# SHI-Labs/Prompt-Free-Diffusion

Hardware: AMD Instinct MI355X
Metric: images/sec @512x512 50-step DDIM, SD-v1.5+SeeCoder (higher is better)
Workload: dtype f16; 1 GPU; [c2] SD-v1.5 UNet + seecoder-v1-0, 512x512, 50-step DDIM (50 real steps), CFG 2.0, fp16, batch=4/GPU, 1 SeeCoder encode(s) + VAE decode per batch; global_batch=4, parallelism=dp1, world_size_reported_by_backend=1, collectives_forced_at_world_1=False

## Files before the change

include/pfd_hip.h:

```cpp
#ifndef PFD_HIP_H
#define PFD_HIP_H

#include <stddef.h>
#include <stdint.h>

#ifdef __cplusplus
extern "C" {
#endif

#define PFD_OK 0
#define PFD_EINVAL (-1)
#define PFD_ESHAPE (-2)
#define PFD_ELAUNCH (-3)

#define PFD_ABI_VERSION 10

typedef void* pfd_stream_t;

#define PFD_ACT_NONE 0
#define PFD_ACT_GELU 1
#define PFD_ACT_RELU 2
#define PFD_ACT_SILU 3
#define PFD_ACT_GEGLU 4

// ... 11 lines not shown
  int32_t M, N, K;
  int32_t rows_per_rv;
  int32_t act;
  int32_t bias_per_row;
  int32_t ksize, stride, pad, ups;
  int32_t B, H, Wd, Cin;
  int32_t Ho, Wo;
  void* ws;
  size_t ws_bytes;
  void* Ct;
  int64_t ldct;
  int32_t n_split;
  int32_t w_tiled;
  const void* gn_table;
  const void* A2;
  int64_t lda2;
  int32_t gn_c1;
  int32_t gn_act;
  const void* ln_stats;
  const void* ln_colsum;
  int32_t ln_parts;
  float ln_eps;
  void* ln_out;
  int32_t k_split;
  int32_t zero_rows;
  void* gn_out;
  const void* gnf_gamma;
  const void* gnf_beta;
  void* gnf_y;
  int64_t gnf_ldy;
  float gnf_eps;
  int32_t gnf_act;
  int32_t gnf_rows;
  int32_t gnf_skip_raw;
  int32_t res_rows;
} PfdGemmDesc;
int pfd_gemm_f16(const PfdGemmDesc* d, pfd_stream_t stream);
int pfd_gemm_f16_ex(const PfdGemmDesc* d, int32_t tile, pfd_stream_t stream);

int32_t pfd_gemm_geglu_group(int32_t N);

typedef struct PfdAttnDesc {
  const void* Q;
  const void* K;
  const void* Vt;
  void* O;
  int64_t ldq, ldk, ldvt, ldo;
  int64_t q_bs, k_bs, vt_bs, o_bs;
  int32_t B, H, Nq, Nk, D;
  float scale;
} PfdAttnDesc;
int pfd_attention_f16(const PfdAttnDesc* d, pfd_stream_t stream);

typedef struct PfdSwinAttnDesc {
  const void* qkv;
  const void* qkv_bias;
  const void* rpb;
  void* out;
  int32_t B, H, W, C, nH, ws, shift;
  float scale;
} PfdSwinAttnDesc;
int pfd_swin_window_attention_f16(const PfdSwinAttnDesc* d, pfd_stream_t stream);

size_t pfd_groupnorm_ws_bytes(int32_t B, int32_t C, int32_t HW);
int32_t pfd_groupnorm_takes_pstats(int32_t B, int32_t C1, int32_t C2, int32_t HW, int32_t G);
int pfd_groupnorm_pstats_f16(const void* x1, int32_t C1, int64_t ldx1, const void* st1, const void* x2, int32_t C2,
                             int64_t ldx2, const void* st2, const void* gamma, const void* beta, void* y, int64_t ldy,
                             int32_t B, int32_t HW, int32_t G, float eps, int32_t act, pfd_stream_t stream);

int pfd_groupnorm_table_f16(const void* x1, int32_t C1, int64_t ldx1, const void* x2, int32_t C2, int64_t ldx2,
                            const void* gamma, const void* beta, void* table, int32_t B, int32_t HW, int32_t G,
                            float eps, void* ws, size_t ws_bytes, pfd_stream_t stream);
int pfd_groupnorm_f16(const void* x1, int32_t C1, int64_t ldx1, const void* x2, int32_t C2,
                      int64_t ldx2, const void* gamma, const void* beta, void* y, int64_t ldy,
                      int32_t B, int32_t HW, int32_t G, float eps, int32_t act ,
                      void* ws, size_t ws_bytes, pfd_stream_t stream);

int pfd_layernorm_f16(const void* x, int64_t ldx, const void* gamma, const void* beta, void* y,
                      int64_t ldy, int32_t M, int32_t C, float eps, int32_t gather4, int32_t B,
                      int32_t H, int32_t W, pfd_stream_t stream);

int pfd_ln_rowstats_f16(const void* x, int64_t ldx, int32_t M, int32_t C, void* out, pfd_stream_t stream);

int pfd_softmax_rows_f16(const void* x, int64_t ldx, void* y, int64_t ldy, int32_t R, int32_t N,
                         float scale, pfd_stream_t stream);

int pfd_nchw_to_nhwc_f16(const void* x, int32_t src_f32, void* y, int32_t B, int32_t C, int32_t H,
                         int32_t W, float mul, float add, int32_t rep, pfd_stream_t stream);
int pfd_nhwc_to_nchw(const void* x, void* y, int32_t dst_f32, int32_t B, int32_t C, int32_t H,
                     int32_t W, float mul, float add, float lo, float hi, pfd_stream_t stream);
int pfd_im2col_f16(const void* x, int64_t ldx, void* col, int32_t B, int32_t H, int32_t W,
                   int32_t Cin, int32_t ksize, int32_t stride, int32_t pad, int32_t Ho, int32_t Wo,
                   int32_t Kpad, pfd_stream_t stream);
int pfd_timestep_embedding_f16(const int64_t* t, void* out, int32_t B, int32_t dim,
                               float max_period, pfd_stream_t stream);
int pfd_cfg_ddim_step(const void* eps, int32_t nb, const float* x, const float* noise,
                      const float* coef, float* x_prev, float* pred_x0, void* xin_next, int32_t rep,
                      int32_t B, int32_t C, int32_t h, int32_t w, pfd_stream_t stream);
int pfd_philox_normal_f32(const int64_t* key, int32_t step, float* out, int32_t B, int64_t n_per_sample,
                          pfd_stream_t stream);
int pfd_cfg_ddim_step_rng(const void* eps, int32_t nb, const float* x, const int64_t* key, int32_t step,
                          float noise_mul, const float* coef, float* x_prev, float* pred_x0, void* xin_next,
                          int32_t rep, int32_t B, int32_t C, int32_t h, int32_t w, pfd_stream_t stream);
int pfd_cfg_ddim_step_ps(const void* eps, int32_t nb, const float* x, const float* noise, const int64_t* key,
                         int32_t step, float noise_mul, const float* coef, const float* scale, float* x_prev,
                         float* pred_x0, void* xin_next, int32_t rep, int32_t B, int32_t C, int32_t h, int32_t w,
// ... 41 lines not shown
```

prompt-free-diffusion_amd/csrc/capi.hip:

```cpp
#include <string.h>

#include "pfd_common.h"

static thread_local char g_err[256] = "";

void pfd_set_error(const char* msg) {
  strncpy(g_err, msg ? msg : "", sizeof(g_err) - 1);
  g_err[sizeof(g_err) - 1] = 0;
}

int pfd_check_launch(const char* what) {
  hipError_t e = hipGetLastError();
  if (e == hipSuccess) return PFD_OK;
  char buf[256];
  snprintf(buf, sizeof(buf), "%s: %s", what, hipGetErrorString(e));
  pfd_set_error(buf);
  return PFD_ELAUNCH;
}

extern "C" int pfd_abi_version(void) { return PFD_ABI_VERSION; }
extern "C" const char* pfd_last_error(void) { return g_err; }

#include <mutex>
#include <vector>

namespace {
constexpr int kProfBuckets = 22;
constexpr int kProfRing = 16384;
struct ProfSlot {
  hipEvent_t a = nullptr, b = nullptr;
  int bucket = -1;
};
struct ProfState {
  bool on = false;
  std::vector<ProfSlot> ring;
  size_t head = 0;
  double ms[kProfBuckets] = {0};
  double flops[kProfBuckets] = {0};
  double bytes[kProfBuckets] = {0};
  long launches[kProfBuckets] = {0};
  int open_slot = -1;
};
ProfState g_prof;
std::mutex g_prof_mu;
const char* kBucketNames[kProfBuckets] = {
    "gemm_conv_kernel<1,1,false>", "gemm_conv_kernel<1,2,false>", "gemm_conv_kernel<2,1,false>",
    "gemm_conv_kernel<2,2,false>", "gemm_conv_kernel<1,1,true>",  "gemm_conv_kernel<1,2,true>",
    "gemm_conv_kernel<2,1,true>",  "gemm_conv_kernel<2,2,true>",  "attention_kernel",
    "swin_attn_kernel",            "groupnorm(stats+finalize+apply)", "layernorm_kernel",
    "gemm160_kernel<4,4>(256x160)", "gemm160_kernel<2,4>(128x160)", "gemm160_kernel<2,2>(64x160)",
    "elementwise / glue",          "gemm160_kernel<4,4,conv>(256x160)", "gemm160_kernel<2,4,conv>(128x160)",
    "gemm160_kernel<2,2,conv>(64x160)", "conv3x3_patch_kernel(256x160)", "conv3x3_narrow_kernel(N<=16)",
    "splitk_reduce(+epilogue / GroupNorm)"};

void harvest(ProfSlot& s) {
  if (s.bucket < 0) return;
  float t = 0.f;
  if (hipEventSynchronize(s.b) == hipSuccess && hipEventElapsedTime(&t, s.a, s.b) == hipSuccess)
    g_prof.ms[s.bucket] += t;
  s.bucket = -1;
}
}

bool pfd_prof_on() { return g_prof.on; }

void pfd_prof_begin(int bucket, double flops, double bytes, hipStream_t stream) {
  std::lock_guard<std::mutex> lk(g_prof_mu);
  if (!g_prof.on || bucket < 0 || bucket >= kProfBuckets) return;
  if (g_prof.ring.empty()) g_prof.ring.resize(kProfRing);
  ProfSlot& s = g_prof.ring[g_prof.head];
  harvest(s);
  if (!s.a) {
    (void)hipEventCreate(&s.a);
    (void)hipEventCreate(&s.b);
  }
  s.bucket = bucket;
  g_prof.flops[bucket] += flops;
  g_prof.bytes[bucket] += bytes;
  g_prof.launches[bucket] += 1;
  g_prof.open_slot = (int)g_prof.head;
  g_prof.head = (g_prof.head + 1) % kProfRing;
  (void)hipEventRecord(s.a, stream);
}

void pfd_prof_end(hipStream_t stream) {
  std::lock_guard<std::mutex> lk(g_prof_mu);
  if (!g_prof.on || g_prof.open_slot < 0) return;
  (void)hipEventRecord(g_prof.ring[g_prof.open_slot].b, stream);
  g_prof.open_slot = -1;
}

extern "C" int pfd_prof_enable(int32_t on) {
  std::lock_guard<std::mutex> lk(g_prof_mu);
  for (auto& s : g_prof.ring) harvest(s);
  for (int i = 0; i < kProfBuckets; ++i) {
    g_prof.ms[i] = g_prof.flops[i] = g_prof.bytes[i] = 0;
    g_prof.launches[i] = 0;
  }
  g_prof.on = on != 0;
  g_prof.open_slot = -1;
  return PFD_OK;
}

extern "C" int pfd_prof_read(int32_t bucket, double* ms, int64_t* launches, double* flops, double* bytes) {
  std::lock_guard<std::mutex> lk(g_prof_mu);
  if (bucket < 0 || bucket >= kProfBuckets) return PFD_EINVAL;
// ... 13 lines not shown
```

prompt-free-diffusion_amd/lib/hip/binding.py:

```python
import ctypes as C
import os

_LIB = None
_LIB_PATH = os.path.normpath(os.path.join(os.path.dirname(os.path.abspath(__file__)), "..", "..", "libpfd_hip.so"))

ABI_VERSION = 10

ACT_NONE, ACT_GELU, ACT_RELU, ACT_SILU, ACT_GEGLU = 0, 1, 2, 3, 4

_i32, _i64, _f32, _vp, _sz = C.c_int32, C.c_int64, C.c_float, C.c_void_p, C.c_size_t


class PfdGemmDesc(C.Structure):
    _fields_ = [
        ("A", _vp), ("W", _vp), ("bias", _vp), ("rowvec", _vp), ("R", _vp), ("C", _vp),
        ("lda", _i64), ("ldw", _i64), ("ldr", _i64), ("ldc", _i64), ("ldrv", _i64),
        ("M", _i32), ("N", _i32), ("K", _i32),
        ("rows_per_rv", _i32), ("act", _i32), ("bias_per_row", _i32),
        ("ksize", _i32), ("stride", _i32), ("pad", _i32), ("ups", _i32),
        ("B", _i32), ("H", _i32), ("Wd", _i32), ("Cin", _i32), ("Ho", _i32), ("Wo", _i32),
        ("ws", _vp), ("ws_bytes", _sz),
        ("Ct", _vp), ("ldct", _i64), ("n_split", _i32), ("w_tiled", _i32),
        ("gn_table", _vp), ("A2", _vp), ("lda2", _i64), ("gn_c1", _i32), ("gn_act", _i32),
        ("ln_stats", _vp), ("ln_colsum", _vp), ("ln_parts", _i32), ("ln_eps", _f32), ("ln_out", _vp),
        ("k_split", _i32), ("zero_rows", _i32), ("gn_out", _vp),
        ("gnf_gamma", _vp), ("gnf_beta", _vp), ("gnf_y", _vp), ("gnf_ldy", _i64), ("gnf_eps", _f32), ("gnf_act", _i32),
        ("gnf_rows", _i32), ("gnf_skip_raw", _i32), ("res_rows", _i32),
    ]


class PfdAttnDesc(C.Structure):
    _fields_ = [
        ("Q", _vp), ("K", _vp), ("Vt", _vp), ("O", _vp),
        ("ldq", _i64), ("ldk", _i64), ("ldvt", _i64), ("ldo", _i64),
        ("q_bs", _i64), ("k_bs", _i64), ("vt_bs", _i64), ("o_bs", _i64),
        ("B", _i32), ("H", _i32), ("Nq", _i32), ("Nk", _i32), ("D", _i32),
        ("scale", _f32),
    ]


class PfdSwinAttnDesc(C.Structure):
    _fields_ = [
        ("qkv", _vp), ("qkv_bias", _vp), ("rpb", _vp), ("out", _vp),
        ("B", _i32), ("H", _i32), ("W", _i32), ("C", _i32), ("nH", _i32), ("ws", _i32), ("shift", _i32),
        ("scale", _f32),
    ]


SIGNATURES = {
    "pfd_abi_version": (_i32, []),
    "pfd_last_error": (C.c_char_p, []),
    "pfd_gemm_f16": (_i32, [C.POINTER(PfdGemmDesc), _vp]),
    "pfd_gemm_f16_ex": (_i32, [C.POINTER(PfdGemmDesc), _i32, _vp]),
    "pfd_gemm_geglu_group": (_i32, [_i32]),
    "pfd_attention_f16": (_i32, [C.POINTER(PfdAttnDesc), _vp]),
    "pfd_swin_window_attention_f16": (_i32, [C.POINTER(PfdSwinAttnDesc), _vp]),
    "pfd_groupnorm_ws_bytes": (_sz, [_i32, _i32, _i32]),
    "pfd_groupnorm_table_f16": (_i32, [_vp, _i32, _i64, _vp, _i32, _i64, _vp, _vp, _vp, _i32, _i32, _i32, _f32, _vp, _sz,
                                       _vp]),
    "pfd_groupnorm_f16": (_i32, [_vp, _i32, _i64, _vp, _i32, _i64, _vp, _vp, _vp, _i64, _i32, _i32, _i32, _f32,
                                 _i32, _vp, _sz, _vp]),
    "pfd_groupnorm_takes_pstats": (_i32, [_i32, _i32, _i32, _i32, _i32]),
    "pfd_groupnorm_pstats_f16": (_i32, [_vp, _i32, _i64, _vp, _vp, _i32, _i64, _vp, _vp, _vp, _vp, _i64, _i32, _i32, _i32,
                                        _f32, _i32, _vp]),
    "pfd_layernorm_f16": (_i32, [_vp, _i64, _vp, _vp, _vp, _i64, _i32, _i32, _f32, _i32, _i32, _i32, _i32, _vp]),
    "pfd_ln_rowstats_f16": (_i32, [_vp, _i64, _i32, _i32, _vp, _vp]),
    "pfd_softmax_rows_f16": (_i32, [_vp, _i64, _vp, _i64, _i32, _i32, _f32, _vp]),
    "pfd_nchw_to_nhwc_f16": (_i32, [_vp, _i32, _vp, _i32, _i32, _i32, _i32, _f32, _f32, _i32, _vp]),
    "pfd_nhwc_to_nchw": (_i32, [_vp, _vp, _i32, _i32, _i32, _i32, _i32, _f32, _f32, _f32, _f32, _vp]),
    "pfd_im2col_f16": (_i32, [_vp, _i64, _vp, _i32, _i32, _i32, _i32, _i32, _i32, _i32, _i32, _i32, _i32, _vp]),
    "pfd_timestep_embedding_f16": (_i32, [_vp, _vp, _i32, _i32, _f32, _vp]),
    "pfd_cfg_ddim_step": (_i32, [_vp, _i32, _vp, _vp, _vp, _vp, _vp, _vp, _i32, _i32, _i32, _i32, _i32, _vp]),
    "pfd_philox_normal_f32": (_i32, [_vp, _i32, _vp, _i32, _i64, _vp]),
    "pfd_cfg_ddim_step_rng": (_i32, [_vp, _i32, _vp, _vp, _i32, _f32, _vp, _vp, _vp, _vp, _i32, _i32, _i32, _i32, _i32,
                                     _vp]),
    "pfd_cfg_ddim_step_ps": (_i32, [_vp, _i32, _vp, _vp, _vp, _i32, _f32, _vp, _vp, _vp, _vp, _vp, _i32, _i32, _i32, _i32,
                                    _i32, _vp]),
    "pfd_add_f16": (_i32, [_vp, _vp, _vp, _i64, _vp]),
    "pfd_axpby_f16": (_i32, [_vp, _f32, _vp, _f32, _vp, _i64, _vp]),
    "pfd_add_rowvec_f16": (_i32, [_vp, _i64, _vp, _vp, _i64, _i32, _i32, _vp]),
    "pfd_add_rowvec_lnstats_f16": (_i32, [_vp, _i64, _vp, _vp, _i64, _i32, _i32, _vp, _vp]),
    "pfd_act_f16": (_i32, [_vp, _vp, _i64, _i32, _vp]),
    "pfd_image_u8_f16": (_i32, [_vp, _vp, _i64, _f32, _f32, _i32, _vp]),
    "pfd_image_resample_check": (_i32, [_i32, _i32, _i32, _i32, _i32, _i32]),
    "pfd_image_resample_h_u8": (_i32, [_vp, _vp, _i32, _i32, _i32, _i32, _i32, _vp, _vp, _vp, _i32, _vp]),
    "pfd_image_resample_v_u8": (_i32, [_vp, _vp, _i32, _i32, _i32, _i32, _i32, _i32, _vp, _vp, _vp, _i32, _vp]),
    "pfd_prof_enable": (_i32, [_i32]),
    "pfd_prof_read": (_i32, [_i32, C.POINTER(C.c_double), C.POINTER(_i64), C.POINTER(C.c_double),
                             C.POINTER(C.c_double)]),
    "pfd_prof_bucket_name": (C.c_char_p, [_i32]),
    "pfd_prof_num_buckets": (_i32, []),
}


def lib_path():
    return os.environ.get("PFD_HIP_LIB", _LIB_PATH)


def load():
    global _LIB
    if _LIB is not None:
        return _LIB
    path = lib_path()
    if not os.path.exists(path):
        raise RuntimeError(
            f"libpfd_hip.so not found at {path}: build it with `python __graft_entry__.py` "
            "(or `make -C prompt-free-diffusion_amd/csrc`).  There is no CPU/torch fallback.")
    lib = C.CDLL(path)
# ... 44 lines not shown
```

prompt-free-diffusion_amd/lib/hip/layers.py:

```python
import torch
import torch.nn as nn

from . import ops
from .ops import ACT_GEGLU, ACT_GELU, ACT_NONE, ACT_RELU, ACT_SILU


def _round_up(v, m):
    return (v + m - 1) // m * m


_GENERATION = [0]


def generation():
    return _GENERATION[0]


def invalidate_packed(module=None):
    _GENERATION[0] += 1
    if module is not None:
        for m in module.modules():
            m.__dict__.pop("_pk_cache", None)


# ... 13 lines not shown
    w = _dev16(w2d)
    N, K = w.shape
    Kp = _round_up(K, kpad_to)
    if Kp != K:
        wp = torch.zeros((N, Kp), dtype=torch.float16, device=w.device)
        wp[:, :K] = w
        return wp
    return w.contiguous()


def pack_conv_weight(w4d):
    w = _dev16(w4d)
    Cout = w.shape[0]
    return pack_matrix(w.permute(0, 2, 3, 1).reshape(Cout, -1))


_UPS_TAPS = (((0,), (1, 2)), ((0, 1), (2,)))


def pack_conv_weight_ups(w4d, dtype=torch.float16):
    w = w4d.detach()
    w = w if w.dtype == torch.float64 else w.float()
    Cout, Cin = w.shape[:2]
    if tuple(w.shape[2:]) != (3, 3):
        raise ValueError(f"pack_conv_weight_ups: a 3x3 kernel, got {tuple(w4d.shape)}")
    blocks = []
    for py in range(2):
        for px in range(2):
            taps = []
            for ty in range(2):
                for tx in range(2):
                    acc = None
                    for ky in _UPS_TAPS[py][ty]:
                        for kx in _UPS_TAPS[px][tx]:
                            acc = w[:, :, ky, kx] if acc is None else acc + w[:, :, ky, kx]
                    taps.append(acc)
            blocks.append(torch.stack(taps, 1).reshape(Cout, 4 * Cin))
    return torch.stack(blocks, 0).to(dtype).contiguous()


def pack_vec(b):
    return None if b is None else _dev16(b).contiguous()


def fold_layernorm(w, b, gamma, beta):
    w32 = w.float()
    g32, be32 = gamma.detach().float(), beta.detach().float()
    wg = (w32 * g32[None, :]).to(torch.float16).contiguous()
    cs = wg.float().sum(1).contiguous()
    bp = (w32 * be32[None, :]).sum(1)
    if b is not None:
        bp = bp + b.float()
    return wg, cs, bp.to(torch.float16).contiguous()


class _Packed:

    def _packed(self, name, builder, *params):
        cache = self.__dict__.setdefault("_pk_cache", {})
        sig = _sig(*params)
        ent = cache.get(name)
        if ent is None or ent[0] != sig:
            with torch.no_grad():
                ent = (sig, builder())
            cache[name] = ent
        return ent[1]


def _io_wrap_nchw(mod, x, fn):
    y = fn(ops.to_nhwc(x))
    return ops.to_nchw(y, x.dtype if x.dtype in (torch.float16, torch.float32) else torch.float32)


class Conv2d(nn.Conv2d, _Packed):

    def _pk(self):
        return self._packed("w", lambda: (pack_conv_weight(self.weight), pack_vec(self.bias)), self.weight, self.bias)

    def _pk_ups(self):
        return self._packed("w_ups", lambda: (pack_conv_weight_ups(self.weight), pack_vec(self.bias)), self.weight, self.bias)

    def hip_gn(self, x, norm, *, silu=True, keep_raw=False, rowvec=None, res=None, rows_per_rv=None):
        k, s, p = self.kernel_size[0], self.stride[0], self.padding[0]
        if self.in_channels % 64 or k != 3 or norm.num_groups != 32 or norm.num_channels != self.out_channels:
            return None
        w, b = self._pk()
        g, be = norm._pk()
        return ops.conv(x, w, k, stride=s, pad=p, bias=b, rowvec=rowvec, res=res, rows_per_rv=rows_per_rv,
                        gn_fuse=(g, be, norm.eps, silu, keep_raw))

    def hip(self, x, *, ups=False, rowvec=None, res=None, act=ACT_NONE, out=None, out_hw=None, rows_per_rv=None,
            gn=None, ln_out=None, gn_out=False, res_rows=None):
        k, s, p = self.kernel_size[0], self.stride[0], self.padding[0]
        cin = self.in_channels
        ln_out = ops.ln_out_arg(ln_out)
        if ups and ops.UPS_FOLD and gn is None and cin % 64 == 0 and (k, s, p) == (3, 1, 1) and rowvec is None and res is None and out_hw is None \
                and ln_out is None and res_rows is None:
            key = ops.ups_fold_key(x, self.out_channels, act, self.bias, out, gn_out)
            if not ops.ups_fold_declined(key):
                wf, b = self._pk_ups()
                y = ops.conv(x, wf, k, ups=2, bias=b, act=act, out=out, gn_out=gn_out)
                if y is not None:
                    return y
                self.__dict__.get("_pk_cache", {}).pop("w_ups", None)
        w, b = self._pk()
        if gn is not None:
# ... 146 lines not shown
```

prompt-free-diffusion_amd/lib/hip/ops.py:

```python
import ctypes as C
import functools
import os
import threading

import torch

from . import binding as _b
from .binding import ACT_GEGLU, ACT_GELU, ACT_NONE, ACT_RELU, ACT_SILU

_byref = C.byref


def _lib():
    return _b.load()


def _stream():
    return torch.cuda.current_stream().cuda_stream


def _ptr(t):
    return t.data_ptr() if t is not None else None


# ... 375 lines not shown
    if not _launch(d, tile, f"pfd_gemm_f16(conv{form}) M{M} N{N} K{K}" + (" with GroupNorm prologue" if gn is not None else ""),
                   fold_key if phase else None):
        return None
    return _written(out, gst)


def im2col(x, ksize, stride, pad, kpad, ho=None, wo=None):
    _chk16(x, "im2col x")
    B, H, W_, Cin = x.shape
    Ho = (H + 2 * pad - ksize) // stride + 1 if ho is None else ho
    Wo = (W_ + 2 * pad - ksize) // stride + 1 if wo is None else wo
    col = torch.empty((B * Ho * Wo, kpad), dtype=torch.float16, device=x.device)
    rc = _lib().pfd_im2col_f16(x.data_ptr(), x.stride(2), col.data_ptr(), B, H, W_, Cin, ksize, stride, pad,
                               Ho, Wo, kpad, _stream())
    _b.check(rc, "pfd_im2col_f16")
    return col, Ho, Wo


def conv_narrow(x, w, ksize, *, stride=1, pad=None, bias=None, rowvec=None, res=None, act=ACT_NONE,
                ho=None, wo=None, out=None, gn_out=False):
    if pad is None:
        pad = ksize // 2
    B = x.shape[0]
    col, Ho, Wo = im2col(x, ksize, stride, pad, w.shape[1], ho, wo)
    N = w.shape[0]
    o2 = None if out is None else out.view(-1, out.shape[-1])
    gn_out = bool(gn_out) and gn_stats_wanted(B, Ho * Wo, N) and wide_tile_ok(N, w.shape[1])
    y = gemm(col, w, bias=bias, rowvec=rowvec, rows_per_rv=Ho * Wo, res=res, act=act, out=o2, gn_out=gn_out)
    r = y.view(B, Ho, Wo, N) if out is None else out
    return _written(r, get_gn_stats(y) if gn_out else None)


def attention(q, k, vt, B, H, Nq, Nk, D, scale, *, ldq, ldk, ldvt, q_bs, k_bs, vt_bs, out=None):
    _chk16(q, "attention q")
    _chk16(k, "attention k")
    _chk16(vt, "attention vt")
    if out is None:
        out = torch.empty((B * Nq, H * D), dtype=torch.float16, device=q.device)
    else:
        _chk16(out, "attention out")
        if out.device != q.device or out.dim() != 2 or out.shape[0] < B * Nq or out.shape[1] < H * D or out.stride(-2) % 8:
            raise ValueError(f"attention: out {tuple(out.shape)} strides {out.stride()} on {out.device} is not a matrix of at "
                             f"least [{B * Nq}, {H * D}] with a row stride that is a multiple of 8 on {q.device}")
    d = _b.PfdAttnDesc()
    d.Q, d.K, d.Vt, d.O = q.data_ptr(), k.data_ptr(), vt.data_ptr(), out.data_ptr()
    d.ldq, d.ldk, d.ldvt, d.ldo = ldq, ldk, ldvt, out.stride(-2)
    d.q_bs, d.k_bs, d.vt_bs, d.o_bs = q_bs, k_bs, vt_bs, Nq * out.stride(-2)
    d.B, d.H, d.Nq, d.Nk, d.D = B, H, Nq, Nk, D
    d.scale = scale
    _b.check(_lib().pfd_attention_f16(_byref(d), _stream()), f"pfd_attention_f16 B{B} H{H} Nq{Nq} Nk{Nk} D{D}")
    return out


def swin_window_attention(qkv, qkv_bias, rpb, B, H, W_, Cdim, nH, ws, shift, scale, out=None):
    _chk16(qkv, "swin qkv")
    if out is None:
        out = torch.empty((B * H * W_, Cdim), dtype=torch.float16, device=qkv.device)
    else:
        _chk16(out, "swin out")
        if out.device != qkv.device or tuple(out.shape) != (B * H * W_, Cdim) or not out.is_contiguous():
            raise ValueError(f"swin_window_attention: out {tuple(out.shape)} on {out.device} is not a dense "
                             f"[{B * H * W_}, {Cdim}] on {qkv.device}")
    d = _b.PfdSwinAttnDesc()
    d.qkv, d.qkv_bias, d.rpb, d.out = qkv.data_ptr(), qkv_bias.data_ptr(), rpb.data_ptr(), out.data_ptr()
    d.B, d.H, d.W, d.C, d.nH, d.ws, d.shift = B, H, W_, Cdim, nH, ws, shift
    d.scale = scale
    _b.check(_lib().pfd_swin_window_attention_f16(_byref(d), _stream()), "pfd_swin_window_attention_f16")
    return _written(out)


def groupnorm(x, gamma, beta, groups, eps, *, x2=None, silu=False, out=None):
    _chk16(x, "groupnorm x")
    B = x.shape[0]
    C1 = x.shape[-1]
    HW = x.numel() // (B * C1)
    C2 = 0 if x2 is None else x2.shape[-1]
    if out is None:
        out = torch.empty(tuple(x.shape[:-1]) + (C1 + C2,), dtype=torch.float16, device=x.device)
    lib = _lib()
    st1 = get_gn_stats(x) if GN_PSTATS else None
    st2 = get_gn_stats(x2) if (GN_PSTATS and x2 is not None) else None
    if _TRACE_GN:
        with open(_TRACE_GN, "a") as f:
            f.write(f"{B} {HW} {C1} {C2} {int(st1 is not None)} {int(x2 is None or st2 is not None)} "
                    f"{int(bool(lib.pfd_groupnorm_takes_pstats(B, C1, C2, HW, groups)))}\n")
    if st1 is not None and (x2 is None or st2 is not None) and groups == 32 and \
            lib.pfd_groupnorm_takes_pstats(B, C1, C2, HW, groups):
        rc = lib.pfd_groupnorm_pstats_f16(x.data_ptr(), C1, x.stride(-2), st1.data_ptr(), _ptr(x2), C2,
                                          0 if x2 is None else x2.stride(-2), _ptr(st2), gamma.data_ptr(), beta.data_ptr(),
                                          out.data_ptr(), out.stride(-2), B, HW, groups, eps,
                                          ACT_SILU if silu else ACT_NONE, _stream())
        _b.check(rc, f"pfd_groupnorm_pstats_f16 B{B} HW{HW} C{C1}+{C2}")
        return _written(out)
    wsb = lib.pfd_groupnorm_ws_bytes(B, C1 + C2, HW)
    ws = torch.empty(wsb, dtype=torch.uint8, device=x.device)
    rc = lib.pfd_groupnorm_f16(x.data_ptr(), C1, x.stride(-2), _ptr(x2), C2, 0 if x2 is None else x2.stride(-2),
                               gamma.data_ptr(), beta.data_ptr(), out.data_ptr(), out.stride(-2), B, HW, groups,
                               eps, ACT_SILU if silu else ACT_NONE, ws.data_ptr(), wsb, _stream())
    _b.check(rc, f"pfd_groupnorm_f16 B{B} HW{HW} C{C1}+{C2}")
    return _written(out)


def groupnorm_table(x, gamma, beta, groups, eps, *, x2=None):
    _chk16(x, "groupnorm_table x")
    B = x.shape[0]
    C1 = x.shape[-1]
# ... 256 lines not shown
```

prompt-free-diffusion_amd/lib/model_zoo/attention.py:

```python
import numpy as np
import numpy.random as npr
import torch
import torch.nn as nn

from ..hip import binding
from ..hip import layers as L
from ..hip import ops


def exists(v):
    return v is not None


def default(v, d):
    return v if v is not None else (d() if callable(d) else d)


def Normalize(in_channels):
    return L.GroupNorm(num_groups=32, num_channels=in_channels, eps=1e-6, affine=True)


class ContextKV:

    def __init__(self, context):
# ... 94 lines not shown
        project_in = GEGLU(dim, inner_dim) if glu else nn.Sequential(L.Linear(dim, inner_dim), nn.GELU())
        self.net = nn.Sequential(project_in, nn.Dropout(dropout), L.Linear(inner_dim, dim_out))

    def hip(self, x2d, res=None, ln=None):
        if self.glu:
            h = self.net[0].hip(x2d, ln=ln)
        else:
            h = self.net[0][0].hip(x2d, act=ops.ACT_GELU, ln=ln)
        return self.net[2].hip(h, res=res)

    def forward(self, x):
        y = self.hip(x.to(torch.float16).reshape(-1, x.shape[-1]))
        return y.view(*x.shape[:-1], y.shape[-1]).to(x.dtype)


class CrossAttention(nn.Module, L._Packed):
    def __init__(self, query_dim, context_dim=None, heads=8, dim_head=64, dropout=0.):
        super().__init__()
        inner_dim = dim_head * heads
        context_dim = default(context_dim, query_dim)
        self.scale = dim_head ** -0.5
        self.heads = heads
        self.dim_head = dim_head
        self.inner_dim = inner_dim
        self.to_q = L.Linear(query_dim, inner_dim, bias=False)
        self.to_k = L.Linear(context_dim, inner_dim, bias=False)
        self.to_v = L.Linear(context_dim, inner_dim, bias=False)
        self.to_out = nn.Sequential(L.Linear(inner_dim, query_dim), nn.Dropout(dropout))

    def _pk_qk(self):
        return self._packed(
            "qk", lambda: torch.cat([L._dev16(self.to_q.weight), L._dev16(self.to_k.weight)], 0).contiguous(),
            self.to_q.weight, self.to_k.weight)

    def _pk_qkv(self):
        return self._packed(
            "qkv", lambda: torch.cat([L._dev16(self.to_q.weight), L._dev16(self.to_k.weight),
                                      L._dev16(self.to_v.weight)], 0).contiguous(),
            self.to_q.weight, self.to_k.weight, self.to_v.weight)

    def _pk_qkv_ln(self, norm):
        def build():
            w = torch.cat([L._dev16(self.to_q.weight), L._dev16(self.to_k.weight), L._dev16(self.to_v.weight)], 0)
            return L.fold_layernorm(w.contiguous(), None, norm.weight, norm.bias)
        return self._packed("qkv_ln", build, self.to_q.weight, self.to_k.weight, self.to_v.weight, norm.weight, norm.bias)

    def ln_foldable(self, x, N, context):
        Cd = self.inner_dim
        if not ops.ln_fold_ok(x.shape[1]):
            return False
        if context is None:
            return N % 8 == 0 and Cd % 160 == 0 and x.shape[1] % 64 == 0
        return Cd % 160 == 0 or Cd % 128 == 0

    def hip(self, x, B, N, context=None, res=None, ln=None, stats_out=False, single=False):
        Cd, H, D = self.inner_dim, self.heads, self.dim_head
        if ln is not None and not self.ln_foldable(x, N, context):
            raise ValueError("CrossAttention.hip: ln= passed for a shape the fold does not serve (see ln_foldable)")
        if context is None:
            if N % 8 == 0 and Cd % 160 == 0 and x.shape[1] % 64 == 0:
                Np = N
                vt = torch.empty((Cd, B * N), dtype=torch.float16, device=x.device)
                if ln is not None:
                    norm, st = ln
                    wq, cs, bq = self._pk_qkv_ln(norm)
                    qk = ops.gemm(x, wq, bias=bq, out_t=vt, n_split=2 * Cd, ln=(st, cs, norm.eps))
                else:
                    qk = ops.gemm(x, self._pk_qkv(), out_t=vt, n_split=2 * Cd)
            elif N % 8 == 0:
                Np = N
                qk = ops.gemm(x, self._pk_qk())
                vt = self.to_v.hip_t(x)
            else:
                qk = ops.gemm(x, self._pk_qk())
                Np = (N + 7) // 8 * 8
                vt = torch.zeros((Cd, B * Np), dtype=torch.float16, device=x.device)
                for b in range(B):
                    self.to_v.hip_t(x[b * N:(b + 1) * N], out=vt[:, b * Np:b * Np + N])
            o = ops.attention(qk, qk[:, Cd:], vt, B, H, N, N, D, self.scale, ldq=2 * Cd, ldk=2 * Cd,
                              ldvt=B * Np, q_bs=N * 2 * Cd, k_bs=N * 2 * Cd, vt_bs=Np)
        else:
            k, vt = context.get(self)
            if context.B != B:
                raise ValueError(f"context batch {context.B} != activation batch {B}")
            z = context.zero_lead
            if single:
                if not (res is not None and 2 * z == B and stats_out and ops.wide_tile_ok(self.to_out[0].out_features, Cd)):
                    raise ValueError("CrossAttention.hip(single=True) needs the zero-context shortcut on half the batch, a residual, "
                                     "statistics and the wide-tile out-projection (SpatialTransformer.hip checks before it asks)")
                w_o, b_o = self.to_out[0]._pk()
                out = torch.empty((B * N, res.shape[1]), dtype=torch.float16, device=res.device)
                st_o = torch.empty((B * N, out.shape[1] // 160, 2), dtype=torch.float32, device=out.device)
                q = self.to_q.hip(x, ln=ln)
                o = ops.attention(q, k[z * context.Nkp:], vt[:, z * context.Nkp:], B - z, H, N, context.Nk, D,
                                  self.scale, ldq=Cd, ldk=Cd, ldvt=B * context.Nkp, q_bs=N * Cd,
                                  k_bs=context.Nkp * Cd, vt_bs=context.Nkp)
                ops.gemm(o, w_o, bias=b_o, res=res, out=out, zero_rows=z * N, ln_out=st_o, res_rows=z * N)
                return out, st_o
            if 0 < z < B and res is not None:
                Bc = B - z
                out = torch.empty_like(res)
                w_o, b_o = self.to_out[0]._pk()
                st_o = None
                if stats_out:
                    st_o = torch.empty((B * N, out.shape[1] // 160, 2), dtype=torch.float32, device=out.device)
                q = self.to_q.hip(x[z * N:], ln=None if ln is None else (ln[0], ln[1][z * N:]))
                o = ops.attention(q, k[z * context.Nkp:], vt[:, z * context.Nkp:], Bc, H, N, context.Nk, D,
                                  self.scale, ldq=Cd, ldk=Cd, ldvt=B * context.Nkp, q_bs=N * Cd,
                                  k_bs=context.Nkp * Cd, vt_bs=context.Nkp)
                if ops.wide_tile_ok(w_o.shape[0], Cd):
                    ops.gemm(o, w_o, bias=b_o, res=res, out=out, zero_rows=z * N, ln_out=st_o)
                    return (out, st_o) if stats_out else out
                ops.add_rowvec(res[:z * N], b_o, out=out[:z * N], ln_out=None if st_o is None else st_o[:z * N])
                if stats_out:
                    self.to_out[0].hip(o, res=res[z * N:], out=out[z * N:], ln_out=st_o[z * N:])
                    return out, st_o
                self.to_out[0].hip(o, res=res[z * N:], out=out[z * N:])
                return out
            q = self.to_q.hip(x, ln=ln)
            o = ops.attention(q, k, vt, B, H, N, context.Nk, D, self.scale, ldq=Cd, ldk=Cd,
                              ldvt=B * context.Nkp, q_bs=N * Cd, k_bs=context.Nkp * Cd, vt_bs=context.Nkp)
        return self.to_out[0].hip(o, res=res, ln_out=True if stats_out else None)

    def forward(self, x, context=None, mask=None):
        assert mask is None, "mask is not supported on the HIP path"
        B, N, _ = x.shape
        ctx = None if context is None else as_context_kv(context)
        y = self.hip(x.to(torch.float16).reshape(B * N, -1), B, N, ctx)
        return y.view(B, N, -1).to(x.dtype)


class BasicTransformerBlock(nn.Module):
    def __init__(self, dim, n_heads, d_head, dropout=0., context_dim=None, gated_ff=True, checkpoint=True,
                 disable_self_attn=False):
        super().__init__()
        self.disable_self_attn = disable_self_attn
        self.attn1 = CrossAttention(query_dim=dim, heads=n_heads, dim_head=d_head, dropout=dropout,
                                    context_dim=context_dim if disable_self_attn else None)
# ... 126 lines not shown
```

Before: 8.074 images/s.

## Fuse cross-attention to_q, attention and to_out into one kernel for C=320

Adds a single HIP kernel that, for 320-channel cross-attention blocks, runs the LayerNorm-folded Q projection, flash-style attention over the short context, the output projection with bias and residual, and the LayerNorm row statistics. Each block keeps a 64-row tile in LDS and streams prepacked weights through a register ring. This replaces separate GEMM, attention and GEMM launches and their intermediate global-memory round trips. It only applies to C=320, 8 heads of 40 and Nk<=256. It also handles zero-context samples by copying the input plus bias. It is enabled by default through an environment flag.

```diff
diff --git a/include/pfd_hip.h b/include/pfd_hip.h
--- a/include/pfd_hip.h
+++ b/include/pfd_hip.h
@@ -87,6 +87,27 @@
 } PfdAttnDesc;
 int pfd_attention_f16(const PfdAttnDesc* d, pfd_stream_t stream);
 
+typedef struct PfdCrossBlockDesc {
+  const void* x;
+  const void* ln_stats;
+  const void* wq;
+  const void* ln_colsum;
+  const void* bq;
+  const void* K;
+  const void* Vt;
+  const void* wo;
+  const void* bo;
+  void* out;
+  void* ln_out;
+  int64_t ldx, ldk, ldvt, k_bs, vt_bs, ldo;
+  int32_t B, zero_samples, N, C, H, D, Nk;
+  int32_t single;
+  float scale;
+  float ln_eps;
+} PfdCrossBlockDesc;
+int32_t pfd_cross_attention_block_takes(const PfdCrossBlockDesc* d);
+int pfd_cross_attention_block_f16(const PfdCrossBlockDesc* d, pfd_stream_t stream);
+
 typedef struct PfdSwinAttnDesc {
   const void* qkv;
   const void* qkv_bias;
diff --git a/prompt-free-diffusion_amd/csrc/capi.hip b/prompt-free-diffusion_amd/csrc/capi.hip
--- a/prompt-free-diffusion_amd/csrc/capi.hip
+++ b/prompt-free-diffusion_amd/csrc/capi.hip
@@ -25,7 +25,7 @@
 #include <vector>
 
 namespace {
-constexpr int kProfBuckets = 22;
+constexpr int kProfBuckets = 23;
 constexpr int kProfRing = 16384;
 struct ProfSlot {
   hipEvent_t a = nullptr, b = nullptr;
@@ -51,7 +51,7 @@
     "gemm160_kernel<4,4>(256x160)", "gemm160_kernel<2,4>(128x160)", "gemm160_kernel<2,2>(64x160)",
     "elementwise / glue",          "gemm160_kernel<4,4,conv>(256x160)", "gemm160_kernel<2,4,conv>(128x160)",
     "gemm160_kernel<2,2,conv>(64x160)", "conv3x3_patch_kernel(256x160)", "conv3x3_narrow_kernel(N<=16)",
-    "splitk_reduce(+epilogue / GroupNorm)"};
+    "splitk_reduce(+epilogue / GroupNorm)", "attention_cross_block_kernel(to_q+attn+to_out)"};
 
 void harvest(ProfSlot& s) {
   if (s.bucket < 0) return;
diff --git a/prompt-free-diffusion_amd/csrc/cross_block.hip b/prompt-free-diffusion_amd/csrc/cross_block.hip
--- /dev/null
+++ b/prompt-free-diffusion_amd/csrc/cross_block.hip
@@ -0,0 +1,367 @@
+#include "pfd_common.h"
+
+namespace {
+
+constexpr int CB_C = 320, CB_H = 8, CB_D = 40, CB_BM = 64, CB_NT = 512;
+constexpr int CB_LD = CB_C + 8;
+constexpr int CB_PROF_BUCKET = 22;
+
+struct CrossParams {
+  const half_t* x;
+  const float* xs;
+  const half_t* wq;
+  const float* cs;
+  const half_t* bq;
+  const half_t* K;
+  const half_t* Vt;
+  const half_t* wo;
+  const half_t* bo;
+  half_t* out;
+  float* so;
+  long ldx, ldk, ldvt, k_bs, vt_bs, ldo;
+  int N, Nk, z, single;
+  float c;
+  float eps;
+};
+
+template <class T>
+__device__ __forceinline__ T cb_gld(const void* ptr) {
+  return *reinterpret_cast<const __attribute__((address_space(1))) T*>((unsigned long)ptr);
+}
+template <class T>
+__device__ __forceinline__ void cb_gst(void* ptr, T v) {
+  *reinterpret_cast<__attribute__((address_space(1))) T*>((unsigned long)ptr) = v;
+}
+__device__ __forceinline__ half8_t cb_cat(half4_t a, half4_t b) { return __builtin_shufflevector(a, b, 0, 1, 2, 3, 4, 5, 6, 7); }
+
+constexpr int CB_KC = 4, CB_NCH = CB_C / 16 / CB_KC, CB_RING = 3;
+__device__ __forceinline__ void cb_wload(const half_t* Wp, int w, int ch, int lane, half8_t (&a)[CB_KC][2]) {
+  const int l1 = 64 + (lane >> 5) * 8 + (lane & 7);
+#pragma unroll
+  for (int kk = 0; kk < CB_KC; ++kk) {
+    const half_t* b = Wp + (long)((w * (CB_C / 16) + ch * CB_KC + kk) * 80) * 8;
+    a[kk][0] = cb_gld<half8_t>(b + lane * 8);
+    a[kk][1] = cb_gld<half8_t>(b + l1 * 8);
+  }
+  __builtin_amdgcn_sched_barrier(0);
+}
+__device__ __forceinline__ void cb_proj(const half_t* Wp, int w, const half_t* Bs, int lane, half8_t (&a)[CB_RING][CB_KC][2],
+                                        float16_t (&acc)[2][2]) {
+  const half_t* b0 = Bs + (lane & 31) * CB_LD + (lane >> 5) * 8;
+  const half_t* b1 = b0 + 32 * CB_LD;
+#pragma unroll
+  for (int ch = 0; ch < CB_NCH; ++ch) {
+    if (ch + 2 < CB_NCH) cb_wload(Wp, w, ch + 2, lane, a[(ch + 2) % CB_RING]);
+#pragma unroll
+    for (int kk = 0; kk < CB_KC; ++kk) {
+      const int ks = ch * CB_KC + kk;
+      const half8_t x0 = *reinterpret_cast<const half8_t*>(b0 + ks * 16);
+      const half8_t x1 = *reinterpret_cast<const half8_t*>(b1 + ks * 16);
+      acc[0][0] = __builtin_amdgcn_mfma_f32_32x32x16_f16(a[ch % CB_RING][kk][0], x0, acc[0][0], 0, 0, 0);
+      acc[0][1] = __builtin_amdgcn_mfma_f32_32x32x16_f16(a[ch % CB_RING][kk][0], x1, acc[0][1], 0, 0, 0);
+      acc[1][0] = __builtin_amdgcn_mfma_f32_32x32x16_f16(a[ch % CB_RING][kk][1], x0, acc[1][0], 0, 0, 0);
+      acc[1][1] = __builtin_amdgcn_mfma_f32_32x32x16_f16(a[ch % CB_RING][kk][1], x1, acc[1][1], 0, 0, 0);
+    }
+  }
+}
+
+struct CbKV {
+  half4_t k[5];
+  half4_t v[2][2][2];
+};
+
+__global__ __launch_bounds__(CB_NT) void cross_block_kernel(const CrossParams p) {
+  __shared__ __attribute__((aligned(16))) half_t lds[2 * CB_BM * CB_LD];
+  half_t* const xsm = lds;
+  half_t* const osm = lds + CB_BM * CB_LD;
+
+  const int tid = threadIdx.x, lane = tid & 63, w = tid >> 6;
+  const int l31 = lane & 31, hi = lane >> 5;
+  const int nblk = gridDim.x;
+  const int blk = xcd_remap(blockIdx.x, nblk);
+  const int tps = p.N / CB_BM;
+  const int smp = blk / tps;
+  const int r0 = (blk - smp * tps) * CB_BM;
+  const long x_row0 = (long)(p.single ? smp : p.z + smp) * p.N + r0;
+  const long o_row0 = (long)(p.z + smp) * p.N + r0;
+
+  const int prow = tid >> 3, psl = (tid >> 2) & 1, pk = tid & 3;
+  const int pcol = psl * 160 + pk * 8;
+  auto row_store = [&](const half8_t (&v)[5], const bool add_bias, long m) __attribute__((always_inline)) {
+    float sum = 0.f, sq = 0.f;
+#pragma unroll
+    for (int j = 0; j < 5; ++j) {
+      half8_t o = v[j];
+      if (add_bias) {
+        const half8_t b = cb_gld<half8_t>(p.bo + pcol + j * 32);
+#pragma unroll
+        for (int e = 0; e < 8; ++e) o[e] = (half_t)((float)v[j][e] + (float)b[e]);
+      }
+#pragma unroll
+      for (int e = 0; e < 8; ++e) {
+        const float f = (float)o[e];
+        sum += f;
+        sq = fmaf(f, f, sq);
+      }
+      cb_gst<half8_t>(p.out + m * p.ldo + pcol + j * 32, o);
+    }
+    sum += __shfl_xor(sum, 1, 64);
+    sq += __shfl_xor(sq, 1, 64);
+    sum += __shfl_xor(sum, 2, 64);
+    sq += __shfl_xor(sq, 2, 64);
+    if (pk == 0) {
+      typedef float f2 __attribute__((ext_vector_type(2)));
+      cb_gst<f2>(p.so + (m * 2 + psl) * 2, (f2){sum, sq});
+    }
+  };
+
+  half8_t wa[CB_RING][CB_KC][2];
+  cb_wload(p.wq, w, 0, lane, wa[0]);
+  cb_wload(p.wq, w, 1, lane, wa[1]);
+  {
+    half8_t xv[5];
+    const half_t* xp = p.x + (x_row0 + prow) * p.ldx + pcol;
+#pragma unroll
+    for (int j = 0; j < 5; ++j) xv[j] = cb_gld<half8_t>(xp + j * 32);
+#pragma unroll
+    for (int j = 0; j < 5; ++j) *reinterpret_cast<half8_t*>(xsm + prow * CB_LD + pcol + j * 32) = xv[j];
+    if (p.single) {
+      row_store(xv, true, x_row0 + prow);
+    } else {
+      const int nz = p.z * tps;
+      for (int ch = blk; ch < nz; ch += nblk) {
+        const long m = (long)ch * CB_BM + prow;
+        half8_t zv[5];
+#pragma unroll
+        for (int j = 0; j < 5; ++j) zv[j] = cb_gld<half8_t>(p.x + m * p.ldx + pcol + j * 32);
+        row_store(zv, true, m);
+      }
+    }
+  }
+  __syncthreads();
+
+  const half_t* Kb = p.K + (long)smp * p.k_bs + w * CB_D + 4 * hi;
+  const half_t* Vb = p.Vt + (long)smp * p.vt_bs;
+  const long vrow[2] = {(long)(w * CB_D + l31) * p.ldvt, (long)(w * CB_D + min(32 + l31, CB_D - 1)) * p.ldvt};
+  const int Nk = p.Nk, nk8 = (Nk + 7) & ~7;
+  const int nkt = (Nk + 31) >> 5;
+  const float c = p.c;
+  auto load_kv = [&](int kv0, CbKV& f) __attribute__((always_inline)) {
+    const half_t* kp = Kb + (long)min(kv0 + l31, Nk - 1) * p.ldk;
+#pragma unroll
+    for (int i = 0; i < 5; ++i) f.k[i] = cb_gld<half4_t>(kp + i * 8);
+#pragma unroll
+    for (int t = 0; t < 2; ++t)
+#pragma unroll
+      for (int s = 0; s < 2; ++s)
+#pragma unroll
+        for (int u = 0; u < 2; ++u) {
+          const int c0 = kv0 + 16 * s + 8 * u + 4 * hi;
+          half4_t v = cb_gld<half4_t>(Vb + vrow[t] + min(c0, nk8 - 4));
+#pragma unroll
+          for (int e = 0; e < 4; ++e)
+            if (c0 + e >= Nk) v[e] = (half_t)0.f;
+          f.v[t][s][u] = v;
+        }
+  };
+  CbKV cur;
+  load_kv(0, cur);
+
+  half8_t qf[2][3];
+  {
+    float16_t acc[2][2];
+#pragma unroll
+    for (int t = 0; t < 2; ++t)
+#pragma unroll
+      for (int mt = 0; mt < 2; ++mt)
+#pragma unroll
+        for (int r = 0; r < 16; ++r) acc[t][mt][r] = 0.f;
+    cb_proj(p.wq, w, xsm, lane, wa, acc);
+#pragma unroll
+    for (int mt = 0; mt < 2; ++mt) {
+      const float4_t st = cb_gld<float4_t>(p.xs + (x_row0 + mt * 32 + l31) * 4);
+      const float sum = st[0] + st[2], sq = st[1] + st[3];
+      const float inv_k = 1.0f / (float)CB_C;
+      const float mean = sum * inv_k;
+      const float var = fmaxf(fmaf(-mean, mean, sq * inv_k), 0.f);
+      const float rstd = rsqrtf(var + p.eps);
+      const float nrm = -rstd * mean;
+      half_t qh[2][16];
+#pragma unroll
+      for (int t = 0; t < 2; ++t)
+#pragma unroll
+        for (int g = 0; g < (t == 0 ? 4 : 1); ++g) {
+          const int n = w * CB_D + t * 32 + g * 8 + hi * 4;
+          const float4_t csv = cb_gld<float4_t>(p.cs + n);
+          const half4_t bv = cb_gld<half4_t>(p.bq + n);
+#pragma unroll
+          for (int e = 0; e < 4; ++e)
+            qh[t][g * 4 + e] = (half_t)(fmaf(acc[t][mt][g * 4 + e], rstd, nrm * csv[e]) + (float)bv[e]);
+        }
+#pragma unroll
+      for (int j = 0; j < 8; ++j) {
+        qf[mt][0][j] = qh[0][j];
+        qf[mt][1][j] = qh[0][8 + j];
+        qf[mt][2][j] = j < 4 ? qh[1][j] : (half_t)0.f;
+      }
+    }
+  }
+
+  {
+    float16_t o[2][2];
+    float m_run[2], l_run[2];
+#pragma unroll
+    for (int qs = 0; qs < 2; ++qs) {
+      m_run[qs] = -INFINITY;
+      l_run[qs] = 0.f;
+#pragma unroll
+      for (int t = 0; t < 2; ++t)
+#pragma unroll
+        for (int r = 0; r < 16; ++r) o[qs][t][r] = 0.f;
+    }
+    CbKV nxt;
+    for (int kt = 0; kt < nkt; ++kt) {
+      const int kv0 = kt * 32;
+      load_kv(min(kv0 + 32, (nkt - 1) * 32), nxt);
+      const half4_t z4 = (half4_t){(half_t)0.f, (half_t)0.f, (half_t)0.f, (half_t)0.f};
+      const half8_t kf0 = cb_cat(cur.k[0], cur.k[1]), kf1 = cb_cat(cur.k[2], cur.k[3]), kf2 = cb_cat(cur.k[4], z4);
+#pragma unroll
+      for (int qs = 0; qs < 2; ++qs) {
+        float16_t st;
+#pragma unroll
+        for (int r = 0; r < 16; ++r) st[r] = 0.f;
+        st = __builtin_amdgcn_mfma_f32_32x32x16_f16(kf0, qf[qs][0], st, 0, 0, 0);
+        st = __builtin_amdgcn_mfma_f32_32x32x16_f16(kf1, qf[qs][1], st, 0, 0, 0);
+        st = __builtin_amdgcn_mfma_f32_32x32x16_f16(kf2, qf[qs][2], st, 0, 0, 0);
+        float mx = -INFINITY;
+#pragma unroll
+        for (int r = 0; r < 16; ++r) {
+          if (kv0 + mfma32_row(r, hi) >= Nk) st[r] = -INFINITY;
+          mx = fmaxf(mx, st[r]);
+        }
+        mx = fmaxf(mx, __shfl_xor(mx, 32, 64));
+        const float m_new = fmaxf(m_run[qs], mx);
+        const float alpha = __builtin_amdgcn_exp2f((m_run[qs] - m_new) * c);
+        m_run[qs] = m_new;
+        const float mc = m_new * c;
+        float rs = 0.f;
+        half8_t pf[2];
+#pragma unroll
+        for (int s = 0; s < 2; ++s)
+#pragma unroll
+          for (int j = 0; j < 8; ++j) {
+            const half_t ph = (half_t)__builtin_amdgcn_exp2f(fmaf(st[s * 8 + j], c, -mc));
+            rs += (float)ph;
+            pf[s][j] = ph;
+          }
+        rs += __shfl_xor(rs, 32, 64);
+        l_run[qs] = fmaf(l_run[qs], alpha, rs);
+#pragma unroll
+        for (int t = 0; t < 2; ++t) {
+#pragma unroll
+          for (int r = 0; r < 16; ++r) o[qs][t][r] *= alpha;
+#pragma unroll
+          for (int s = 0; s < 2; ++s)
+            o[qs][t] = __builtin_amdgcn_mfma_f32_32x32x16_f16(cb_cat(cur.v[t][s][0], cur.v[t][s][1]), pf[s], o[qs][t], 0, 0, 0);
+        }
+      }
+      cur = nxt;
+    }
+    cb_wload(p.wo, w, 0, lane, wa[0]);
+    cb_wload(p.wo, w, 1, lane, wa[1]);
+#pragma unroll
+    for (int qs = 0; qs < 2; ++qs) {
+      const float inv = 1.0f / l_run[qs];
+      half_t* op = osm + (qs * 32 + l31) * CB_LD + w * CB_D + hi * 4;
+#pragma unroll
+      for (int t = 0; t < 2; ++t)
+#pragma unroll
+        for (int g = 0; g < (t == 0 ? 4 : 1); ++g) {
+          half4_t v;
+#pragma unroll
+          for (int e = 0; e < 4; ++e) v[e] = (half_t)(o[qs][t][g * 4 + e] * inv);
+          *reinterpret_cast<half4_t*>(op + t * 32 + g * 8) = v;
+        }
+    }
+  }
+  __syncthreads();
+
+  {
+    float16_t acc[2][2];
+#pragma unroll
+    for (int t = 0; t < 2; ++t)
+#pragma unroll
+      for (int mt = 0; mt < 2; ++mt)
+#pragma unroll
+        for (int r = 0; r < 16; ++r) acc[t][mt][r] = 0.f;
+    cb_proj(p.wo, w, osm, lane, wa, acc);
+#pragma unroll
+    for (int t = 0; t < 2; ++t)
+#pragma unroll
+      for (int g = 0; g < (t == 0 ? 4 : 1); ++g) {
+        const int n = w * CB_D + t * 32 + g * 8 + hi * 4;
+        const half4_t bv = cb_gld<half4_t>(p.bo + n);
+#pragma unroll
+        for (int mt = 0; mt < 2; ++mt) {
+          half4_t* xp = reinterpret_cast<half4_t*>(xsm + (mt * 32 + l31) * CB_LD + n);
+          const half4_t xr = *xp;
+          half4_t v;
+#pragma unroll
+          for (int e = 0; e < 4; ++e) v[e] = (half_t)(acc[t][mt][g * 4 + e] + (float)bv[e] + (float)xr[e]);
+          *xp = v;
+        }
+      }
+  }
+  __syncthreads();
+
+  {
+    half8_t rv[5];
+#pragma unroll
+    for (int j = 0; j < 5; ++j) rv[j] = *reinterpret_cast<const half8_t*>(xsm + prow * CB_LD + pcol + j * 32);
+    row_store(rv, false, o_row0 + prow);
+  }
+}
+
+bool cb_takes(const PfdCrossBlockDesc* d) {
+  if (!d) return false;
+  if (d->C != CB_C || d->H != CB_H || d->D != CB_D) return false;
+  if (d->N <= 0 || d->N % CB_BM) return false;
+  if (d->Nk < 1 || d->Nk > 256) return false;
+  if (d->B < 1 || d->zero_samples < 0 || d->zero_samples >= d->B) return false;
+  if (d->single && 2 * d->zero_samples != d->B) return false;
+  if ((long)d->B * d->N > (1L << 30)) return false;
+  if (d->ldx < CB_C || d->ldo < CB_C || d->ldk < CB_C) return false;
+  if ((d->ldx & 7) || (d->ldo & 7) || (d->ldk & 7) || (d->ldvt & 7) || (d->k_bs & 7) || (d->vt_bs & 7)) return false;
+  if (d->ldvt < ((d->Nk + 7) & ~7)) return false;
+  return true;
+}
+
+}
+
+extern "C" int32_t pfd_cross_attention_block_takes(const PfdCrossBlockDesc* d) { return cb_takes(d) ? 1 : 0; }
+
+extern "C" int pfd_cross_attention_block_f16(const PfdCrossBlockDesc* d, pfd_stream_t stream) {
+  if (!d || !d->x || !d->ln_stats || !d->wq || !d->ln_colsum || !d->bq || !d->K || !d->Vt || !d->wo || !d->bo || !d->out ||
+      !d->ln_out)
+    return PFD_EINVAL;
+  if (!cb_takes(d)) return PFD_ESHAPE;
+  if (!aligned16(d->x) || !aligned16(d->ln_stats) || !aligned16(d->wq) || !aligned16(d->ln_colsum) || !aligned16(d->bq) ||
+      !aligned16(d->K) || !aligned16(d->Vt) || !aligned16(d->wo) || !aligned16(d->bo) || !aligned16(d->out) ||
+      !aligned16(d->ln_out))
+    return PFD_EINVAL;
+  CrossParams p;
+  p.x = (const half_t*)d->x; p.xs = (const float*)d->ln_stats; p.wq = (const half_t*)d->wq; p.cs = (const float*)d->ln_colsum;
+  p.bq = (const half_t*)d->bq; p.K = (const half_t*)d->K; p.Vt = (const half_t*)d->Vt; p.wo = (const half_t*)d->wo;
+  p.bo = (const half_t*)d->bo; p.out = (half_t*)d->out; p.so = (float*)d->ln_out;
+  p.ldx = d->ldx; p.ldk = d->ldk; p.ldvt = d->ldvt; p.k_bs = d->k_bs; p.vt_bs = d->vt_bs; p.ldo = d->ldo;
+  p.N = d->N; p.Nk = d->Nk; p.z = d->zero_samples; p.single = d->single ? 1 : 0;
+  p.c = d->scale * 1.4426950408889634f;
+  p.eps = d->ln_eps;
+  const int Bc = d->B - d->zero_samples;
+  const double rows = (double)Bc * d->N;
+  hipStream_t s = (hipStream_t)stream;
+  PfdProfScope prof(CB_PROF_BUCKET, rows * (4.0 * CB_C * CB_C + 4.0 * d->Nk * CB_C),
+                    2.0 * CB_C * ((double)d->B * d->N + (d->single ? rows : (double)d->B * d->N)), s);
+  hipLaunchKernelGGL(cross_block_kernel, dim3(Bc * (d->N / CB_BM)), dim3(CB_NT), 0, s, p);
+  return pfd_check_launch("pfd_cross_attention_block_f16");
+}
diff --git a/prompt-free-diffusion_amd/lib/hip/binding.py b/prompt-free-diffusion_amd/lib/hip/binding.py
--- a/prompt-free-diffusion_amd/lib/hip/binding.py
+++ b/prompt-free-diffusion_amd/lib/hip/binding.py
@@ -39,6 +39,16 @@
     ]
 
 
+class PfdCrossBlockDesc(C.Structure):
+    _fields_ = [
+        ("x", _vp), ("ln_stats", _vp), ("wq", _vp), ("ln_colsum", _vp), ("bq", _vp), ("K", _vp), ("Vt", _vp), ("wo", _vp),
+        ("bo", _vp), ("out", _vp), ("ln_out", _vp),
+        ("ldx", _i64), ("ldk", _i64), ("ldvt", _i64), ("k_bs", _i64), ("vt_bs", _i64), ("ldo", _i64),
+        ("B", _i32), ("zero_samples", _i32), ("N", _i32), ("C", _i32), ("H", _i32), ("D", _i32), ("Nk", _i32),
+        ("single", _i32), ("scale", _f32), ("ln_eps", _f32),
+    ]
+
+
 class PfdSwinAttnDesc(C.Structure):
     _fields_ = [
         ("qkv", _vp), ("qkv_bias", _vp), ("rpb", _vp), ("out", _vp),
@@ -54,6 +64,8 @@
     "pfd_gemm_f16_ex": (_i32, [C.POINTER(PfdGemmDesc), _i32, _vp]),
     "pfd_gemm_geglu_group": (_i32, [_i32]),
     "pfd_attention_f16": (_i32, [C.POINTER(PfdAttnDesc), _vp]),
+    "pfd_cross_attention_block_takes": (_i32, [C.POINTER(PfdCrossBlockDesc)]),
+    "pfd_cross_attention_block_f16": (_i32, [C.POINTER(PfdCrossBlockDesc), _vp]),
     "pfd_swin_window_attention_f16": (_i32, [C.POINTER(PfdSwinAttnDesc), _vp]),
     "pfd_groupnorm_ws_bytes": (_sz, [_i32, _i32, _i32]),
     "pfd_groupnorm_table_f16": (_i32, [_vp, _i32, _i64, _vp, _i32, _i64, _vp, _vp, _vp, _i32, _i32, _i32, _f32, _vp, _sz,
diff --git a/prompt-free-diffusion_amd/lib/hip/layers.py b/prompt-free-diffusion_amd/lib/hip/layers.py
--- a/prompt-free-diffusion_amd/lib/hip/layers.py
+++ b/prompt-free-diffusion_amd/lib/hip/layers.py
@@ -89,6 +89,15 @@
     if b is not None:
         bp = bp + b.float()
     return wg, cs, bp.to(torch.float16).contiguous()
+
+
+def pack_cross_weight(w):
+    if tuple(w.shape) != (320, 320):
+        raise ValueError(f"pack_cross_weight: [320, 320] expected, got {tuple(w.shape)}")
+    v = w.reshape(8, 40, 20, 2, 8)
+    full = v[:, :32].permute(0, 2, 3, 1, 4).reshape(8, 20, 64, 8)
+    rest = v[:, 32:].permute(0, 2, 3, 1, 4).reshape(8, 20, 16, 8)
+    return torch.cat([full, rest], 2).contiguous()
 
 
 class _Packed:
diff --git a/prompt-free-diffusion_amd/lib/hip/ops.py b/prompt-free-diffusion_amd/lib/hip/ops.py
--- a/prompt-free-diffusion_amd/lib/hip/ops.py
+++ b/prompt-free-diffusion_amd/lib/hip/ops.py
@@ -451,6 +451,57 @@
     return out
 
 
+CROSS_FUSED = os.environ.get("PFD_CROSS_FUSED", "1") != "0"
+
+
+def _cross_dims(d, B, z, N, C_, H, D, Nk, single):
+    d.B, d.zero_samples, d.N, d.C, d.H, d.D, d.Nk, d.single = B, z, N, C_, H, D, Nk, 1 if single else 0
+    d.ldx = d.ldo = d.ldk = C_
+    d.ldvt = d.vt_bs = (Nk + 7) // 8 * 8
+    return d
+
+
+def cross_block_takes(B, z, N, C_, H, D, Nk, single=False):
+    return bool(_lib().pfd_cross_attention_block_takes(_byref(_cross_dims(_b.PfdCrossBlockDesc(), B, z, N, C_, H, D, Nk, single))))
+
+
+def cross_attention_block(x, stats, wq, colsum, bq, k, vt, wo, bo, *, B, z, N, H, D, Nk, Nkp, scale, eps, single=False,
+                          out=None, ln_out=None):
+    for t, what in ((x, "x"), (wq, "wq"), (bq, "bq"), (k, "k"), (vt, "vt"), (wo, "wo"), (bo, "bo")):
+        _chk16(t, f"cross_attention_block {what}")
+    rows_x, C_, ldx = _rows(x)
+    if C_ % 160 or wq.numel() != C_ * C_ or wo.numel() != C_ * C_ or bq.numel() != C_ or bo.numel() != C_:
+        return None
+    if rows_x != (B - z if single else B) * N:
+        raise ValueError(f"cross_attention_block: x has {rows_x} rows for B {B} z {z} N {N} single {single}")
+    if stats.dtype != torch.float32 or not stats.is_contiguous() or stats.numel() != rows_x * 4:
+        raise ValueError("cross_attention_block: stats must be a contiguous float32 [rows of x, 2, 2]")
+    if colsum.dtype != torch.float32 or not colsum.is_contiguous() or colsum.numel() != C_:
+        raise ValueError("cross_attention_block: column sums must be a contiguous float32 [C]")
+    if not (wq.is_contiguous() and wo.is_contiguous() and bq.is_contiguous() and bo.is_contiguous()):
+        raise ValueError("cross_attention_block: dense weights expected")
+    if out is None:
+        out = torch.empty((B * N, C_), dtype=torch.float16, device=x.device)
+    else:
+        _chk16(out, "cross_attention_block out")
+        if out.device != x.device or out.dim() != 2 or tuple(out.shape) != (B * N, C_):
+            raise ValueError(f"cross_attention_block: out {tuple(out.shape)} on {out.device} is not [{B * N}, {C_}] on {x.device}")
+    so = _row_stats("cross_attention_block: ln_out", "M, C/160, 2", B * N, C_, x.device, ln_out)
+    d = _cross_dims(_b.PfdCrossBlockDesc(), B, z, N, C_, H, D, Nk, single)
+    kc, vc = k[z * Nkp:], vt[:, z * Nkp:]
+    d.x, d.ln_stats, d.wq, d.ln_colsum, d.bq = x.data_ptr(), stats.data_ptr(), wq.data_ptr(), colsum.data_ptr(), bq.data_ptr()
+    d.K, d.Vt, d.wo, d.bo, d.out, d.ln_out = kc.data_ptr(), vc.data_ptr(), wo.data_ptr(), bo.data_ptr(), out.data_ptr(), so.data_ptr()
+    d.ldx, d.ldo, d.ldk, d.ldvt = ldx, out.stride(-2), k.stride(-2), vt.stride(-2)
+    d.k_bs, d.vt_bs = Nkp * k.stride(-2), Nkp
+    d.scale, d.ln_eps = scale, float(eps)
+    rc = _lib().pfd_cross_attention_block_f16(_byref(d), _stream())
+    if rc == _b.PFD_ESHAPE:
+        return None
+    _b.check(rc, f"pfd_cross_attention_block_f16 B{B} z{z} N{N} Nk{Nk}")
+    _written(out)
+    return out, so
+
+
 def swin_window_attention(qkv, qkv_bias, rpb, B, H, W_, Cdim, nH, ws, shift, scale, out=None):
     _chk16(qkv, "swin qkv")
     if out is None:
diff --git a/prompt-free-diffusion_amd/lib/model_zoo/attention.py b/prompt-free-diffusion_amd/lib/model_zoo/attention.py
--- a/prompt-free-diffusion_amd/lib/model_zoo/attention.py
+++ b/prompt-free-diffusion_amd/lib/model_zoo/attention.py
@@ -170,6 +170,26 @@
         if context is None:
             return N % 8 == 0 and Cd % 160 == 0 and x.shape[1] % 64 == 0
         return Cd % 160 == 0 or Cd % 128 == 0
+
+    def _pk_cross(self, norm):
+        def build():
+            wg, cs, bq = L.fold_layernorm(L.pack_matrix(self.to_q.weight), None, norm.weight, norm.bias)
+            lo = self.to_out[0]
+            return L.pack_cross_weight(wg), cs, bq, L.pack_cross_weight(L.pack_matrix(lo.weight)), L.pack_vec(lo.bias)
+        return self._packed("cross", build, self.to_q.weight, self.to_out[0].weight, self.to_out[0].bias, norm.weight, norm.bias)
+
+    def _hip_fused(self, x, B, N, context, res, ln, stats_out, single):
+        if not (ops.CROSS_FUSED and ln is not None and stats_out and res is x and x.dim() == 2):
+            return None
+        z = context.zero_lead
+        if x.shape[1] != self.inner_dim or self.to_out[0].out_features != self.inner_dim or self.to_out[0].bias is None or \
+                not ops.cross_block_takes(B, z, N, self.inner_dim, self.heads, self.dim_head, context.Nk, single):
+            return None
+        norm, st = ln
+        wq, cs, bq, w_o, b_o = self._pk_cross(norm)
+        k, vt = context.get(self)
+        return ops.cross_attention_block(x, st, wq, cs, bq, k, vt, w_o, b_o, B=B, z=z, N=N, H=self.heads, D=self.dim_head,
+                                         Nk=context.Nk, Nkp=context.Nkp, scale=self.scale, eps=norm.eps, single=single)
 
     def hip(self, x, B, N, context=None, res=None, ln=None, stats_out=False, single=False):
         Cd, H, D = self.inner_dim, self.heads, self.dim_head
@@ -202,6 +222,9 @@
             if context.B != B:
                 raise ValueError(f"context batch {context.B} != activation batch {B}")
             z = context.zero_lead
+            fused = self._hip_fused(x, B, N, context, res, ln, stats_out, single)
+            if fused is not None:
+                return fused
             if single:
                 if not (res is not None and 2 * z == B and stats_out and ops.wide_tile_ok(self.to_out[0].out_features, Cd)):
                     raise ValueError("CrossAttention.hip(single=True) needs the zero-context shortcut on half the batch, a residual, "
```

New measurement: 8.114 images/s, median of 6. No clear change (+0.5%).
